# mehta-lab/VisCy

Hardware: AMD Instinct MI355X
Metric: training patches/sec (Z=5, 256x256, 1->2ch UNeXt2) (higher is better)
Workload: dtype bf16; 1 GPU; UNeXt2 2.5D convnextv2_tiny Z=5 256x256 1->2ch, fwd+MixedLoss(0.5,0,0.5)+bwd+AdamW; per_gpu_batch=512, global_batch=512, parallelism=dp1

## Files before the change

### include/vsx.h

```cpp
#ifndef VSX_H
#define VSX_H
#include <stddef.h>
#include <stdint.h>

#ifdef __cplusplus
extern "C" {
#endif

typedef void* vsx_stream_t;

#define VSX_F32 0
#define VSX_BF16 1

int32_t vsx_version(void);
const char* vsx_last_error(void);
const char* vsx_last_kernel(void);
int32_t vsx_set_flag(const char* name, int32_t value);
int32_t vsx_get_flag(const char* name);
int32_t vsx_det_workspace(float* ws, int64_t floats);
int32_t vsx_det_scope(int32_t on);
int32_t vsx_det_active(void);

#define VSX_A_ROWS 0
#define VSX_A_PATCH2 1
// ... 250 lines not shown
    float* dW2, float* db2, float* ws, int64_t ws_floats, int32_t nb, int32_t C, int32_t dtype, vsx_stream_t stream);
int64_t vsx_grn_q_reduce_ws_floats(int32_t nb, int32_t C);
int32_t vsx_mlp_bwd_stats(const void* dout, const void* wimg, const void* g, float* P, float* S, int64_t M, int32_t C, int32_t hw,
    int32_t dtype, vsx_stream_t stream);
int32_t vsx_mlp_bwd_dh(const void* dout, const void* wimg, const void* h, const float* s, const float* t, void* dh, float* ws,
                       int64_t ws_rows, float* colsum, const float* gelu_table, int64_t M, int32_t C, int32_t hw, int32_t dtype,
                       vsx_stream_t stream);
int32_t vsx_mlp_rows_per_workgroup(int32_t C, int32_t hw, int64_t M);
int32_t vsx_mlp_bwd_dh_re(const void* dout, const void* xh, const void* wimg_bwd, const void* wimg_fwd, const float* b1, const float* s,
                          const float* t, void* dh, float* ws, int64_t ws_rows, float* colsum, const float* gelu_table, int64_t M,
                          int32_t C, int32_t hw, int32_t dtype, vsx_stream_t stream);
int32_t vsx_mlp_bwd_dh_ln(const void* dout, const void* y, const float* mean, const float* rstd, const void* wimg_bwd,
                          const void* wimg_fwd, const float* b1, const float* s, const float* t, void* dh, float* ws, int64_t ws_rows,
                          float* colsum2, const float* gelu_table, int64_t M, int32_t C, int32_t hw, int32_t dtype,
                          vsx_stream_t stream);
int32_t vsx_mlp_gelu_table_len(void);
int32_t vsx_mlp_gelu_table(float* tab, vsx_stream_t stream);

int32_t vsx_adamw_advance(const double* cfg, int32_t* step, float* hyper, vsx_stream_t stream);

int32_t vsx_fill_f32(float* p, int64_t n, float value, vsx_stream_t stream);

int32_t vsx_prep_weight(const float* src, void* dst, void* dstT, const float* gamma, int32_t R, int32_t Cs,
    int32_t Tn, int32_t tapmode, int32_t dtype, vsx_stream_t stream);

int32_t vsx_unprep_grad(const float* g, float* dparam, const float* gamma, const float* W, float* dgamma,
    const float* u, const float* beta, const float* rowsub, int32_t R, int32_t Cs, int32_t Tn, int32_t tapmode,
    vsx_stream_t stream);

int32_t vsx_scale_weight_samples(const float* W, const float* s, void* out, int32_t B, int32_t R, int32_t K,
// ... 198 lines not shown
```

### viscy_amd/csrc/api.hip

```cpp
#include <stdarg.h>
#include <stdio.h>
#include <string.h>
#include "vsx_common.h"
#include "../../include/vsx.h"

static thread_local char g_err[512] = "";
thread_local const char* g_vsx_last_kernel = "";
int g_vsx_tn_tr = 1;
int g_vsx_nt_wide = 1;
int g_vsx_nt_fast = 3;
int g_vsx_tn_wide = 1;
int g_vsx_ggb_blocks = 2048;
int g_vsx_tn_rect = 11;
int g_vsx_dw_mfma = 15;
int g_vsx_ln_fblk = 32768;
int g_vsx_ln_bblk = 8192;
int g_vsx_ln_ablk = 512;
int g_vsx_ln_pack = 1;
int g_vsx_nt_stream = 3;
int g_vsx_grn_stream = 2;
int g_vsx_ggb_contig = 1;
int g_vsx_tn_fill = 1;
int g_vsx_tn_want2 = 512;
int g_vsx_tn_p2_rounds = 1;
// ... 56 lines not shown
    {"tn_want", &g_vsx_tn_want, INT32_MIN},       {"tn_p2_rounds", &g_vsx_tn_p2_rounds, INT32_MIN},
    {"tn_want2", &g_vsx_tn_want2, INT32_MIN},     {"tn_fill", &g_vsx_tn_fill, INT32_MIN},
    {"tn_contig", &g_vsx_tn_contig, INT32_MIN},   {"tn_stream", &g_vsx_tn_stream, INT32_MIN},
    {"ln_stream", &g_vsx_ln_stream, INT32_MIN},   {"ggb_blocks", &g_vsx_ggb_blocks, INT32_MIN},
    {"tn_rect", &g_vsx_tn_rect, INT32_MIN},       {"dw_mfma", &g_vsx_dw_mfma, INT32_MIN},
    {"ln_fblk", &g_vsx_ln_fblk, 1},               {"ln_bblk", &g_vsx_ln_bblk, 1},
    {"ln_ablk", &g_vsx_ln_ablk, 1},               {"ln_pack", &g_vsx_ln_pack, INT32_MIN},
    {"mlp_fused", &g_vsx_mlp_fused, INT32_MIN},   {"loss_fused", &g_vsx_loss_fused, INT32_MIN},
    {"mlp_sf32", &g_vsx_mlp_sf32, INT32_MIN},     {"det_reduce", &g_vsx_det_reduce, INT32_MIN},
    {"head_rows", &g_vsx_head_rows, INT32_MIN},   {"head_bps", &g_vsx_head_bps, 0},
};

extern "C" int32_t vsx_set_flag(const char* name, int32_t value) {
  for (const auto& f : g_flags)
    if (name && !strcmp(name, f.name) && value >= f.min) { *f.value = value; return 0; }
  vsx_set_error("vsx_set_flag: unknown flag '%s'", name ? name : "(null)");
  return 1;
}
extern "C" int32_t vsx_get_flag(const char* name) {
  for (const auto& f : g_flags)
    if (name && !strcmp(name, f.name)) return *f.value;
  return -1;
}
```

### viscy_amd/csrc/mlp.hip

```cpp
#include "vsx_common.h"
#include "mfma16.h"
#include "wtasks.h"
#include "../../include/vsx.h"

struct MlpArgs {
  const bf16_t* xh;
  const char* wimg;
  const float* b1;
  const float* grn_s;
  const float* grn_b;
  const float* b2;
  const bf16_t* res;
  const float* rscale;
  bf16_t* out;
  float* colsq;
  bf16_t* hout;
  bf16_t* gout;
  float ln_eps;
  bf16_t* xh_out;
  float* rstd_out;
  float* mean_out;
  const float* ln_mean;
  const float* ln_rstd;
  const bf16_t* tin;
  float* red0;
  float* red1;
  float* ws;
  const float* gtab;
  const bf16_t* xh2;
  const char* wimg2;
  int M, hw;
  int nt;
};

#define MLP_GT_BASE (103 << 7)
#define MLP_GT_LIM (131 << 7)
#define MLP_GT_N (MLP_GT_LIM - MLP_GT_BASE)

__device__ __forceinline__ float mlp_relu(float h) {
  const int b = __float_as_int(h);
  return __int_as_float(b > 0 ? b : 0);
}

__device__ __forceinline__ uint32_t mlp_relu_pair(uint32_t w) {
  typedef short mlp_s16x2 __attribute__((ext_vector_type(2)));
  const mlp_s16x2 z = {0, 0};
  return __builtin_bit_cast(uint32_t, __builtin_elementwise_max(__builtin_bit_cast(mlp_s16x2, w), z));
// ... 3 lines not shown
__device__ unsigned long long g_mlp_ts[8 * 64 * 8];
#define MLP_STAMP(k) do { if (blockIdx.x == gridDim.x / 2 + 7 && lane == 0) g_mlp_ts[(wave * 64 + hs) * 8 + (k)] = __builtin_amdgcn_s_memtime(); } while (0)
#else
#define MLP_STAMP(k) do { } while (0)
#endif

#ifndef MLP_DMA_WAVES
#define MLP_DMA_WAVES 4
#endif

template <int C, int MF, int NW, int MODE>
struct MlpGeom {
  static constexpr int H4 = 4 * C, NHS = H4 / 32, KK = C / 32, NF = C / 16;
  static constexpr int WM = 16 * MF, BM = NW * WM;
  static constexpr int W1_PIECES = 2 * KK, IMG_PIECES = 2 * KK + NF;
  static constexpr bool RE = MODE == 5 || MODE == 7;
  static constexpr int NP = RE ? 2 * W1_PIECES : (MODE != 1 ? W1_PIECES : IMG_PIECES);
  static constexpr int STAGE_BYTES = NP * 1024;
  static constexpr int OB_COLS = MODE == 0 ? 32 : 64;
  static constexpr int OB_RS = OB_COLS * 2 + 16;
  static constexpr int OUT_BYTES = MODE == 2 ? NW * 2 * WM * OB_RS : NW * WM * OB_RS;
  static constexpr bool B1_IN_PADS = MODE == 6;
  static constexpr int VEC_FLOATS = MODE == 1 ? 3 * H4 + C : (MODE == 4 ? 2 * H4 : (RE ? 3 * H4 : (MODE == 3 || B1_IN_PADS ? 4 : H4)));
  static constexpr int RED_FLOATS = MODE == 1 ? 4 : (MODE == 3 || MODE == 7 ? 4 * NW * 32 : 2 * NW * 32);
  static constexpr int GT_FLOATS = (MODE <= 2 || MODE == 6) ? MLP_GT_N : ((MODE == 4 || RE) ? 2 * MLP_GT_N : 4);
  static constexpr int LDS_BYTES = 2 * STAGE_BYTES + OUT_BYTES + (VEC_FLOATS + RED_FLOATS) * 4;
};

template <int C, int MF, int NW, int MODE>
__device__ __forceinline__ void mlp_fused_body(const MlpArgs& a) {
  typedef MlpGeom<C, MF, NW, MODE> G;
  constexpr int H4 = G::H4, NHS = G::NHS, KK = G::KK, NF = G::NF, WM = G::WM;
  constexpr bool STATS = MODE == 0 || MODE == 2 || MODE == 6, STORE = MODE == 2 || MODE == 6, STORE_H = MODE == 2;
  constexpr bool RE = G::RE, LNF = MODE == 7;
  constexpr bool BWD = (MODE >= 3 && MODE <= 5) || MODE == 7, DH = MODE == 4 || RE;
  constexpr int DW = MLP_DMA_WAVES < NW ? MLP_DMA_WAVES : NW;
  __shared__ __attribute__((aligned(1024))) char buf0[G::STAGE_BYTES];
  __shared__ __attribute__((aligned(1024))) char buf1[G::STAGE_BYTES];
  __shared__ __attribute__((aligned(16))) float vec[G::VEC_FLOATS];
  __shared__ __attribute__((aligned(16))) float red[G::RED_FLOATS];
  __shared__ __attribute__((aligned(16))) char obuf[G::OUT_BYTES];
  __shared__ __attribute__((aligned(16))) float gt[G::GT_FLOATS];

  const int tid = threadIdx.x;
  const MfLane ln = mf_lane(tid);
  const int lane = ln.lane, wave = ln.wave, p16 = ln.p16, kq = ln.kq;
  const int m0 = blockIdx.x * G::BM;
  const int b = m0 / a.hw;
  const int row0 = m0 + wave * WM;

// ... 66 lines not shown
  mf_bf16x8 xf[MF][KK];
#pragma unroll
  for (int mf = 0; mf < MF; ++mf)
#pragma unroll
    for (int kk = 0; kk < KK; ++kk)
      xf[mf][kk] = *reinterpret_cast<const mf_bf16x8*>(a.xh + (size_t)(row0 + mf * 16 + p16) * C + kk * 32 + kq * 8);

  mf_bf16x8 xg[RE ? MF : 1][RE ? KK : 1];
  if constexpr (RE) {
#pragma unroll
    for (int mf = 0; mf < MF; ++mf)
#pragma unroll
      for (int kk = 0; kk < KK; ++kk)
        xg[mf][kk] = *reinterpret_cast<const mf_bf16x8*>(a.xh2 + (size_t)(row0 + mf * 16 + p16) * C + kk * 32 + kq * 8);
  }
  setup_to_lds();
  float rsr[LNF ? MF : 1];
  mf_bf16x8 wS, wSl, wMh, wMl;
  if constexpr (LNF) {
#pragma unroll
    for (int mf = 0; mf < MF; ++mf) {
      const size_t rowi = (size_t)(row0 + mf * 16 + p16);
      const float mean = a.ln_mean[rowi], rstd = a.ln_rstd[rowi];
      rsr[mf] = rstd;
#pragma unroll
      for (int kk = 0; kk < KK; ++kk) {
        union { mf_bf16x8 b; uint4 u; } cv;
        cv.b = xg[mf][kk];
        float v[8], o[8];
        unpack<bf16_t>(cv.u, v);
// ... 63 lines not shown
          }
        }
        if constexpr (STORE) {
          if (kq == 0) {
            a.rstd_out[rowi] = rstd;
            if (a.mean_out) a.mean_out[rowi] = mean;
          }
        }
      }
    }
  }

  mf_f32x4 oacc[MODE == 1 ? MF : 1][MODE == 1 ? NF : 1];
  if constexpr (MODE == 1) {
    mfma_zero(oacc);
  }

  auto gemm1 = [&](const char* W, const auto& xfr, mf_f32x4 (&acc)[2][MF]) {
    mfma_zero(acc);
#pragma unroll
    for (int hf = 0; hf < 2; ++hf)
#pragma unroll
      for (int kk = 0; kk < KK; ++kk) {
        const mf_bf16x8 wa = *reinterpret_cast<const mf_bf16x8*>(W + (hf * KK + kk) * 1024);
#pragma unroll
        for (int mf = 0; mf < MF; ++mf) acc[hf][mf] = mfma16(wa, xfr[mf][kk], acc[hf][mf]);
      }
  };
  char* sb = obuf + wave * ((STORE_H ? 2 : 1) * WM * G::OB_RS);
  auto activate = [&](int hs, const mf_f32x4 (&acc)[2][MF], mf_bf16x8 (&zf)[MF]) {
// ... 120 lines not shown
  };
  auto tile_flush = [&](int hs) {
    if constexpr (DH) {
      __builtin_amdgcn_fence(__ATOMIC_RELEASE, "wavefront");
      __builtin_amdgcn_wave_barrier();
#pragma unroll
      for (int i = 0; i < (WM * 8) / 64; ++i) {
        const int idx = lane + 64 * i, row = idx >> 3, ch = idx & 7;
        const uint4 v = *reinterpret_cast<const uint4*>(sb + row * G::OB_RS + ch * 16);
        stvec_stream(a.hout + (size_t)(row0 + row) * H4 + (hs - 1) * 32 + ch * 8, v, (a.nt & 1) != 0);
      }
      __builtin_amdgcn_fence(__ATOMIC_RELEASE, "wavefront");
      __builtin_amdgcn_wave_barrier();
    }
  };
  auto bwd_act = [&](int hs, const mf_f32x4 (&acc)[2][MF], const mf_f32x4 (&hacc)[2][MF], float (&r0)[2][4], float (&r1)[2][4]) {
    if constexpr (BWD) {
#pragma unroll
      for (int hf = 0; hf < 2; ++hf)
#pragma unroll
        for (int r = 0; r < 4; ++r) { r0[hf][r] = 0.f; r1[hf][r] = 0.f; }
      float sv[2][4], tv[2][4], b1v[2][4];
      if constexpr (DH) {
        const float* vb = vec + hs * 32 + kq * 4;
#pragma unroll
        for (int hf = 0; hf < 2; ++hf) {
          const float4 t2 = *reinterpret_cast<const float4*>(vb + hf * 16);
          const float4 t3 = *reinterpret_cast<const float4*>(vb + H4 + hf * 16);
          sv[hf][0] = t2.x; sv[hf][1] = t2.y; sv[hf][2] = t2.z; sv[hf][3] = t2.w;
          tv[hf][0] = t3.x; tv[hf][1] = t3.y; tv[hf][2] = t3.z; tv[hf][3] = t3.w;
          if constexpr (RE) {
            const float4 t4 = *reinterpret_cast<const float4*>(vb + 2 * H4 + hf * 16);
            b1v[hf][0] = t4.x; b1v[hf][1] = t4.y; b1v[hf][2] = t4.z; b1v[hf][3] = t4.w;
          }
        }
      }
#pragma unroll
      for (int mf = 0; mf < MF; ++mf)
#pragma unroll
        for (int hf = 0; hf < 2; ++hf) {
          char* tp = sb + (mf * 16 + p16) * G::OB_RS + ((hs & 1) * 32 + hf * 16 + kq * 4) * 2;
          uint2 tw;
          if constexpr (RE) {
            const vsx_v2f ha = (vsx_v2f){hacc[hf][mf][0], hacc[hf][mf][1]} + (vsx_v2f){b1v[hf][0], b1v[hf][1]};
            const vsx_v2f hc = (vsx_v2f){hacc[hf][mf][2], hacc[hf][mf][3]} + (vsx_v2f){b1v[hf][2], b1v[hf][3]};
            tw.x = f32x2_to_bf16x2_bits(ha.x, ha.y);
            tw.y = f32x2_to_bf16x2_bits(hc.x, hc.y);
          } else {
            tw = *reinterpret_cast<const uint2*>(tp);
          }
          if constexpr (MODE == 3) {
            const float e[4] = {__uint_as_float(tw.x << 16), __uint_as_float(tw.x & 0xFFFF0000u), __uint_as_float(tw.y << 16),
                                __uint_as_float(tw.y & 0xFFFF0000u)};
// ... 16 lines not shown
#pragma unroll
            for (int r = 0; r < 4; r += 2) {
              const uint32_t w = r < 2 ? tw.x : tw.y;
              const float h0 = __uint_as_float(w << 16), h1 = __uint_as_float(w & 0xFFFF0000u);
              const vsx_v2f d2 = {acc[hf][mf][r], acc[hf][mf][r + 1]};
              const vsx_v2f s2 = {sv[hf][r], sv[hf][r + 1]}, t2 = {tv[hf][r], tv[hf][r + 1]};
              const uint32_t Rq = mlp_relu_pair(w);
              const vsx_v2f gv = (vsx_v2f){__uint_as_float(Rq << 16), __uint_as_float(Rq & 0xFFFF0000u)} - (vsx_v2f){tb[r].x, tb[r + 1].x};
              const vsx_v2f cs = {copysignf(tb[r].y, h0), copysignf(tb[r + 1].y, h1)};
              const vsx_v2f dgv = cs + (vsx_v2f){0.5f, 0.5f};
              vsx_v2f rr = (d2 * s2 + gv * t2) * dgv;
              if constexpr (LNF) rr = rr * (vsx_v2f){rsr[mf], rsr[mf]};
              ob[r / 2] = f32x2_to_bf16x2_bits(rr.x, rr.y);
            }
            *reinterpret_cast<uint2*>(tp) = make_uint2(ob[0], ob[1]);
          }
        }
    }
  };

  auto stage_load2 = [&](int s, char* dst) {
    const char* src1 = a.wimg + (size_t)(s + 1) * (G::IMG_PIECES * 1024) + lane * 16;
    const char* src2 = RE ? a.wimg2 + (size_t)(s + 1) * (G::IMG_PIECES * 1024) - G::W1_PIECES * 1024 + lane * 16
                          : a.wimg + (size_t)s * (G::IMG_PIECES * 1024) + lane * 16;
    if (wave >= DW) return;
    for (int p = wave; p < G::NP; p += DW) {
      if ((RE || p < G::W1_PIECES) && s + 1 >= NHS) continue;
      const char* src = p < G::W1_PIECES ? src1 : src2;
      lds_dma16(src + p * 1024, dst + p * 1024);
    }
  };
  auto store_pending = [&](int hs) {
    if constexpr (STORE) {
      __builtin_amdgcn_fence(__ATOMIC_RELEASE, "wavefront");
      __builtin_amdgcn_wave_barrier();
      for (int idx = lane; idx < (STORE_H ? 2 : 1) * WM * 8; idx += 64) {
        const int o = idx / (WM * 8), rem = idx - o * (WM * 8);
        const int row = rem >> 3, ch = rem & 7;
        const uint4 v = *reinterpret_cast<const uint4*>(sb + (o * WM + row) * G::OB_RS + ch * 16);
        bf16_t* dst = (o || !STORE_H ? a.gout : a.hout) + (size_t)(row0 + row) * H4 + (hs - 1) * 32 + ch * 8;
        stvec_stream(dst, v, (a.nt & 1) != 0);
// ... 75 lines not shown
    }
    mf_bf16x8 zf[MF];
    __builtin_amdgcn_sched_barrier(0);
    MLP_STAMP(2);
    gemm1(S, xf, hnxt);
    if constexpr (RE) gemm1(S + G::W1_PIECES * 1024, xg, gnxt);
    __builtin_amdgcn_sched_group_barrier(0x100, 3, 0);
#pragma unroll
    for (int i = 0; i < (RE ? 4 : 2) * KK; ++i) {
      __builtin_amdgcn_sched_group_barrier(0x008, MF, 0);
      __builtin_amdgcn_sched_group_barrier(0x100, 1, 0);
    }
    __builtin_amdgcn_sched_barrier(0);
    MLP_STAMP(3);
    float q0[2][4], q1[2][4];
    if constexpr (RE) bwd_act(hs, hcur, gcur, q0, q1);
    else if constexpr (BWD) bwd_act(hs, hcur, hcur, q0, q1);
    else activate(hs, hcur, zf);
    __builtin_amdgcn_sched_barrier(0);
    MLP_STAMP(4);
    if constexpr (DH) {
      colsum_mfma(hs, red + (hs & 1) * (LNF ? 2 : 1) * NW * 32 + wave * 32);
    } else if constexpr (BWD) {
      float* rw = red + (hs & 1) * 2 * NW * 32 + wave * 32;
#pragma unroll
      for (int hf = 0; hf < 2; ++hf)
#pragma unroll
        for (int r = 0; r < 4; ++r) {
          const float t0 = group_sum<16>(q0[hf][r]);
          if (p16 == 0) rw[hf * 16 + kq * 4 + r] = t0;
          const float t1 = group_sum<16>(q1[hf][r]);
          if (p16 == 0) rw[NW * 32 + hf * 16 + kq * 4 + r] = t1;
        }
    } else if constexpr (STATS) {
      stats_mfma(hs, red + (hs & 1) * NW * 32 + wave * 32);
// ... 43 lines not shown

  if constexpr (BWD) {
    tile_flush(NHS - 1);
    __syncthreads();
    if constexpr (MODE == 3) {
      if (wave == (NHS - 1) % DW) {
        const float* r = red + ((NHS - 1) & 1) * 2 * NW * 32 + (lane >> 5) * NW * 32 + (lane & 31);
        float t = 0.f;
#pragma unroll
        for (int w = 0; w < NW; ++w) t += r[w * 32];
        atomicAdd((lane < 32 ? a.red0 : a.red1) + (size_t)b * H4 + (NHS - 1) * 32 + (lane & 31), t);
      }
    } else {
      ws_row(NHS - 1, true);
    }
    return;
  } else if constexpr (STATS) {
    store_pending(NHS - 1);
    __syncthreads();
    if (wave == (NHS - 1) % DW && lane < 32) {
      const float* r = red + ((NHS - 1) & 1) * NW * 32 + lane;
      float t = 0.f;
#pragma unroll
      for (int w = 0; w < NW; ++w) t += r[w * 32];
      if (a.ws) a.ws[(size_t)blockIdx.x * H4 + (NHS - 1) * 32 + lane] = t;
      else atomicAdd(a.colsq + (size_t)b * H4 + (NHS - 1) * 32 + lane, t);
    }
    return;
  } else {
    const float rs = a.rscale ? a.rscale[b] : 1.f;
// ... 55 lines not shown
__global__ __launch_bounds__(NW * 64, (MODE == 4 && NW == 8 && C == 96 ? 4 : 1)) void mlp_fused_kernel(const MlpArgs a) {
  mlp_fused_body<C, MF, NW, MODE>(a);
}
template <int C, int MF, int NW, int MODE>
__global__ __launch_bounds__(NW * 64, (MODE == 4 && NW == 8 && C == 96 ? 4 : 1)) __attribute__((target("no-packed-fp32-ops")))
void mlp_fused_kernel_sf(const MlpArgs a) {
  mlp_fused_body<C, MF, NW, MODE>(a);
}

__global__ __launch_bounds__(256) void mlp_pack_kernel(const bf16_t* __restrict__ W1, const bf16_t* __restrict__ W2,
                                                       char* __restrict__ img, int C) {
  wt_mlp_pack(blockIdx.x, W1, W2, img, C);
}

struct MlpCfg { int C, MF, NW, modes; };
static inline int mlp_nt() { return (g_vsx_nt_stream >> 2) & 15; }
static const MlpCfg kMlpCfgs[] = {{96, 2, 8, 255}, {192, 2, 8, 255}, {224, 2, 8, 255}, {384, 2, 8, 4 | 8 | 16}};

static const MlpCfg* mlp_cfg(int C, int hw, long M, int mode) {
  for (const MlpCfg& c : kMlpCfgs) {
    const int bm = c.NW * 16 * c.MF;
    if (!(c.modes & (1 << mode))) continue;
    if (c.C == 384 && !(g_vsx_mlp_fused & 4)) continue;
    if ((mode == 5 || mode == 6 || mode == 7) && !(g_vsx_mlp_fused & 64)) continue;
    if (mode == 7 && !(g_vsx_mlp_fused & 128)) continue;
    if (c.C == C && hw % bm == 0 && M % bm == 0) return &c;
  }
  return nullptr;
}

extern "C" int32_t vsx_mlp_supported(int32_t C, int32_t hw, int64_t M, int32_t dtype) {
  return dtype == VSX_BF16 && mlp_cfg(C, hw, M, 0) != nullptr && mlp_cfg(C, hw, M, 1) != nullptr;
}
extern "C" int32_t vsx_mlp_mode_supported(int32_t C, int32_t hw, int64_t M, int32_t mode, int32_t dtype) {
  return dtype == VSX_BF16 && mode >= 0 && mode <= 7 && mlp_cfg(C, hw, M, mode) != nullptr;
}

extern "C" int64_t vsx_mlp_image_bytes(int32_t C) { return (int64_t)(4 * C / 32) * (2 * (C / 32) + C / 16) * 1024; }

extern "C" int32_t vsx_mlp_pack(const void* W1, const void* W2, void* img, int32_t C, vsx_stream_t stream) {
  VSX_CHECK(W1 && W2 && img && C > 0 && C % 32 == 0, "vsx_mlp_pack: bad arguments (C = %d must be a multiple of 32)", C);
  const long total = (long)(4 * C / 32) * (2 * (C / 32) + C / 16) * 64;
  hipLaunchKernelGGL(mlp_pack_kernel, dim3(vsx_cdiv(total, 256)), dim3(256), 0, (hipStream_t)stream, (const bf16_t*)W1,
                     (const bf16_t*)W2, (char*)img, C);
  VSX_LAUNCH_CHECK();
  return 0;
}

template <int C, int MF, int NW, int MODE>
static int mlp_launch(const MlpArgs& a, hipStream_t s) {
  typedef MlpGeom<C, MF, NW, MODE> G;
  if (g_vsx_mlp_sf32 & (1 << MODE)) hipLaunchKernelGGL((mlp_fused_kernel_sf<C, MF, NW, MODE>), dim3(a.M / G::BM), dim3(NW * 64), 0, s, a);
  else hipLaunchKernelGGL((mlp_fused_kernel<C, MF, NW, MODE>), dim3(a.M / G::BM), dim3(NW * 64), 0, s, a);
  VSX_LAUNCH_CHECK();
  return 0;
}

template <int MODE>
static int mlp_dispatch(const MlpCfg* c, const MlpArgs& a, hipStream_t s) {
  if (c->C == 96) return mlp_launch<96, 2, 8, MODE>(a, s);
  if (c->C == 192) return mlp_launch<192, 2, 8, MODE>(a, s);
  if (c->C == 224) return mlp_launch<224, 2, 8, MODE>(a, s);
  if constexpr (MODE <= 1 || MODE >= 5) { vsx_set_error("vsx_mlp: mode %d is built for C <= 224", MODE); return 1; }
  else return mlp_launch<384, 2, 8, MODE>(a, s);
}

static long mlp_det_need(const MlpCfg* c, long M) { return M / (c->NW * 16 * c->MF) * 4 * c->C; }
static int mlp_det_begin(MlpArgs& a, const MlpCfg* c, const char* who) { return vsx_det_take(who, mlp_det_need(c, a.M), &a.ws); }
static int mlp_det_end(const MlpArgs& a, const MlpCfg* c, hipStream_t s) {
  if (!a.ws) return 0;
  const int bm = c->NW * 16 * c->MF;
  return vsx_det_group_sum(a.ws, 4 * c->C, 0, a.colsq, a.M / a.hw, a.hw / bm, 4 * c->C, s);
}

extern "C" int32_t vsx_mlp_gelu_table_len(void) { return 2 * MLP_GT_N; }

__global__ void mlp_gelu_table_kernel(float* __restrict__ tab) {
// ... 132 lines not shown
  return mlp_bwd_dh_run<5>("vsx_mlp_bwd_dh_re", a, s, t, dh, ws, ws_rows, colsum, 4 * C, gtab, M, C, hw, stream);
}

extern "C" int32_t vsx_mlp_bwd_dh_ln(const void* dout, const void* y, const float* mean, const float* rstd, const void* wimg_bwd,
                                     const void* wimg_fwd, const float* b1, const float* s, const float* t, void* dh, float* ws,
                                     int64_t ws_rows, float* colsum2, const float* gtab, int64_t M, int32_t C, int32_t hw,
                                     int32_t dtype, vsx_stream_t stream) {
  VSX_CHECK(dtype == VSX_BF16, "vsx_mlp_bwd_dh_ln: bf16 only");
  VSX_CHECK(dout && y && mean && rstd && wimg_bwd && wimg_fwd && b1 && s && t && dh && ws && colsum2 && gtab && M > 0 && hw > 0,
            "vsx_mlp_bwd_dh_ln: bad arguments");
  MlpArgs a = mlp_bwd_args(dout, wimg_bwd, M, hw);
  a.xh2 = (const bf16_t*)y; a.wimg2 = (const char*)wimg_fwd; a.b1 = b1; a.ln_mean = mean; a.ln_rstd = rstd;
  return mlp_bwd_dh_run<7>("vsx_mlp_bwd_dh_ln", a, s, t, dh, ws, ws_rows, colsum2, 8 * C, gtab, M, C, hw, stream);
}

#ifdef MLP_TS
extern "C" int32_t vsx_debug_mlp_ts(unsigned long long* host_out) {
  return hipMemcpyFromSymbol(host_out, HIP_SYMBOL(g_mlp_ts), sizeof(g_mlp_ts)) == hipSuccess ? 0 : 1;
}
#endif

extern "C" int64_t vsx_mlp_det_floats(int32_t C, int32_t hw, int64_t M, int32_t mode) {
  const MlpCfg* c = mode == 0 || mode == 2 || mode == 6 ? mlp_cfg(C, hw, M, mode) : nullptr;
  return c ? mlp_det_need(c, M) : 0;
}

extern "C" int32_t vsx_mlp_rows_per_workgroup(int32_t C, int32_t hw, int64_t M) {
  const MlpCfg* c = mlp_cfg(C, hw, M, 4);
  return c ? c->NW * 16 * c->MF : 0;
}
// ... 1 lines not shown
```

### viscy_amd/csrc/vsx_common.h

```cpp
#pragma once
#include <hip/hip_runtime.h>
#include <stdint.h>
#include <math.h>
#include <type_traits>

typedef __bf16 bf16_t;

#define VSX_F32 0
#define VSX_BF16 1

void vsx_set_error(const char* fmt, ...);
extern int g_vsx_tn_tr, g_vsx_tn_wide, g_vsx_tn_rect, g_vsx_tn_want, g_vsx_tn_want2, g_vsx_tn_p2_rounds, g_vsx_tn_fill, g_vsx_tn_contig, g_vsx_tn_stream;
extern int g_vsx_nt_wide, g_vsx_nt_fast, g_vsx_nt_stream, g_vsx_nt2;
extern int g_vsx_ln_fblk, g_vsx_ln_bblk, g_vsx_ln_ablk, g_vsx_ln_pack, g_vsx_ln_stream;
extern int g_vsx_grn_stream, g_vsx_ggb_contig, g_vsx_ggb_blocks;
extern int g_vsx_dw_mfma, g_vsx_mlp_fused, g_vsx_mlp_sf32, g_vsx_loss_fused;
extern int g_vsx_head_bps, g_vsx_head_rows, g_vsx_det_reduce;
extern thread_local int g_vsx_det_scope;
static inline bool vsx_det_on() { return g_vsx_det_reduce || g_vsx_det_scope; }
int vsx_det_take(const char* who, long need, float** ws);
int vsx_det_group_sum(const float* ws, int ld, int col0, float* out, int groups, int rows_per_group, int N, hipStream_t s);
extern thread_local const char* g_vsx_last_kernel;
#define VSX_CHECK(cond, ...)            \
  do {                                  \
    if (!(cond)) {                      \
      vsx_set_error(__VA_ARGS__);       \
      return 1;                         \
    }                                   \
  } while (0)
#define VSX_LAUNCH_CHECK()                                               \
  do {                                                                   \
    hipError_t e_ = hipGetLastError();                                   \
// ... 239 lines not shown
```

### viscy_amd/engine_unext2.py

```python

from __future__ import annotations

import os
from collections import namedtuple
from typing import NamedTuple

import torch
from torch import Tensor

from . import _lib as L
from . import ops as hip_ops
from .flat import FlatEngine, engine_apply


class _BlockW:

    __slots__ = ("C", "p", "dw_w", "W1f", "W1fT", "b1f", "W2", "W2T", "v1", "fc2_w", "fc2_b", "grn_w", "grn_b", "dp", "img", "img2", "b2f")


class _ProjW:
    __slots__ = ("cin", "cout", "taps", "ln", "conv", "W", "WT")


FWD_UNFUSED, FWD_PAIR, FWD_FC1 = 0, 1, 2
# ... 67 lines not shown
            self.off += n_al
            return v
        return self._zeros(*shape)


class Engine(FlatEngine):
    name = "UNeXt2"

    def __init__(self, model, ops=None):
        ops = hip_ops if ops is None else ops
        self._hip = ops is hip_ops
        self._mlp_flag = 0
        self.cfg = model.cfg
        self._zeros4c = {}
        self._dp_inject = None
        self._za = None
        self._za_need = {}
        self._prepared_for = None
        self.W = None
        super().__init__(model, ops)

    def _stage_params_rev(self, stage):
        ps = []
        for blk in reversed(list(stage.blocks)):
            if hasattr(blk, "gamma"):
                ps += [blk.gamma, blk.mlp.fc2.weight, blk.mlp.fc2.bias, blk.mlp.fc1.weight, blk.mlp.fc1.bias, blk.norm.weight,
                       blk.norm.bias, blk.conv_dw.weight, blk.conv_dw.bias]
                continue
            ps += [blk.mlp.fc2.weight, blk.mlp.fc2.bias, blk.mlp.grn.weight, blk.mlp.grn.bias, blk.mlp.fc1.weight,
                   blk.mlp.fc1.bias, blk.norm.weight, blk.norm.bias, blk.conv_dw.weight, blk.conv_dw.bias]
# ... 75 lines not shown
        w = _ProjW()
        cout, cin = conv.weight.shape[0], conv.weight.shape[1]
        taps = conv.weight.shape[2] * conv.weight.shape[3]
        w.cin, w.cout, w.taps, w.ln, w.conv = cin, cout, taps, ln, conv
        if cout < 16:
            w.W = w.WT = None
        else:
            w.W, w.WT = o.prep_weight(conv.weight, cout, cin, taps, dt, want=True, want_t=need_bwd)
        return w

    def prepare(self, dt: torch.dtype, need_bwd: bool, mlp_flag: int = 0):
        key = (dt, need_bwd)
        m, cfg, o = self.model, self.cfg, self.ops
        with o.batch():
            W = self._prepare_ops(dt, need_bwd)
        if dt == torch.bfloat16 and mlp_flag:
            bwd_img = need_bwd and bool(mlp_flag & 8)
            with o.batch():
                for _, blocks in list(W["enc"]) + list(W["dec"]):
                    for w in blocks:
                        if any(o.mlp_supported(w.C, 1 << 20, 1 << 20, dt, md) for md in (None, 2, 4)):
                            w.img = o.mlp_pack(w.W1f, w.W2, w.C)
                            if bwd_img:
                                w.img2 = o.mlp_pack(w.W2T, w.W2, w.C)
        self.W = W
        self._prepared_for = key
        return W

    def _prepare_ops(self, dt: torch.dtype, need_bwd: bool):
        m, cfg, o = self.model, self.cfg, self.ops
        W = {"dt": dt}
        sw = m.stem.conv.weight
        co3, K = sw.shape[0], sw[0].numel()
        Dp = cfg["ratio"]
        narrow_stem = cfg.get("head") == "shuffle" and tuple(cfg["stem_kernel"][1:]) == (2, 2)
        if narrow_stem and K % 8 and Dp == 1:
            W["stem_W"], W["stem_b"] = None, m.stem.conv.bias
        elif Dp == 1:
            W["stem_W"], _ = o.prep_weight(sw, co3, K, 1, dt)
# ... 213 lines not shown
                o.transpose_f32(cs, db2, C, 1, True)
            o.matvec_t_add(w.fc2_w, cs, dgb, C, 4 * C)
        else:
            o.gemm("tn", gact, dout, dW2, M, C, 4 * C, 4 * C, C, 4 * C, dtype=dt, pro=L.PRO_GRN, grn_s=s,
                   grn_b=w.grn_b, hw=hw, colsum=db2)
        if w.v1:
            o.layer_scale_unfold(dW2, db2, blk.mlp.fc2.weight, blk.mlp.fc2.bias, blk.gamma, g(blk.mlp.fc2.weight),
                                 g(blk.mlp.fc2.bias), g(blk.gamma))
        ln_re = not plan.keep_xh
        u1 = None
        if ln_re:
            cs2 = self._za.take(2, 4 * C)
            db1f, u1 = cs2[0], cs2[1]
        else:
            db1f = self._za.take(4 * C)
        if fused_bwd:
            img2 = w.img2
            assert img2 is not None
            if fused_bwd == 2 and not stats_in_tn:
                o.mlp_bwd_stats(dout, img2, gact, PS[0], PS[1], M, C, hw)
            if stats_in_tn:
                t = o.grn_bwd_stats(colsq, PS[0], w.grn_w, dgw)
            else:
                t = o.grn_bwd_stats(colsq, PS[0], w.grn_w, dgw, Sb=PS[1], dbeta=dgb)
            if ln_re:
                dz = o.mlp_bwd_dh_ln(dout, y, mean, rstd, img2, w.img, w.b1f, s, t, cs2, M, C, hw)
            elif not plan.keep_h:
                dz = o.mlp_bwd_dh_re(dout, xh, img2, w.img, w.b1f, s, t, db1f, M, C, hw)
            else:
                dz = o.mlp_bwd_dh(dout, img2, h, s, t, db1f, M, C, hw)
        else:
            dz = torch.empty((M, 4 * C), dtype=dt, device=dev)
            o.gemm("nt", dout, w.W2T, dz, M, 4 * C, C, C, C, 4 * C, dtype=dt, epi=L.EPI_DZ, aux=gact, ldx=4 * C, red0=PS[0],
                   red1=PS[1], hw=hw)
            t = o.grn_bwd_stats(colsq, PS[0], w.grn_w, dgw, Sb=PS[1], dbeta=dgb)
            o.grn_gelu_bwd(dz, h, s, t, db1f, M, 4 * C, hw)
        if ln_re:
            xh = y
        dy = o.dgrad_ln_bwd(dz, w.W1fT, xh, rstd, M, C, 4 * C, mean=mean) if self._hip else None
        assert dy is not None or not ln_re
        dxh = None
        if dy is None:
            dxh = torch.empty((M, C), dtype=dt, device=dev)
            o.gemm("nt", dz, w.W1fT, dxh, M, C, 4 * C, 4 * C, 4 * C, C, dtype=dt)
        dW1f = self._za.take(4 * C, C)
        o.gemm("tn", xh, dz, dW1f, M, 4 * C, C, C, 4 * C, C, dtype=dt)
        del dz
        o.unprep_grad(dW1f, g(blk.mlp.fc1.weight), 4 * C, C, 1, gamma=blk.norm.weight, W=blk.mlp.fc1.weight,
                      dgamma=g(blk.norm.weight), u=db1f, beta=blk.norm.bias, rowsub=u1)
        o.matvec_t_add(blk.mlp.fc1.weight, db1f, g(blk.norm.bias), 4 * C, C)
        o.transpose_f32(db1f, g(blk.mlp.fc1.bias), 4 * C, 1, True)
        if dy is None:
            dy = o.ln_bwd(dxh, xh, None, rstd, None, None, None, None, M, C)
        del dxh
# ... 380 lines not shown
```

### viscy_amd/ops.py

```python

from __future__ import annotations

import contextlib
import ctypes as C
import os
import threading
from typing import Sequence

import torch
from torch import Tensor

from . import _lib as L
from ._lib import VsxGemm, VsxGemmPlan, check, dtype_code, lib, ptr, stream


class Scratch:

    def __init__(self, alloc=None):
        self._alloc = alloc or (lambda floats, dev: torch.empty(floats, dtype=torch.float32, device=dev))
        self._tls = threading.local()
        self.held: list = []

    def take(self, dev, floats: int):
        arenas = getattr(self._tls, "arenas", None)
# ... 524 lines not shown
def mlp_bwd_dh(dout: Tensor, img2: Tensor, h: Tensor, s: Tensor, t: Tensor, colsum: Tensor, M: int, C: int, hw: int) -> Tensor:
    dh, ws, rows = _mlp_dh_alloc(dout, M, C, hw, 4 * C)
    check(lib().vsx_mlp_bwd_dh(ptr(dout), ptr(img2), ptr(h), ptr(s), ptr(t), ptr(dh), ptr(ws), rows, ptr(colsum),
                               ptr(_gelu_table(dout.device)), M, C, hw, dtype_code(dout.dtype), stream()), "mlp_bwd_dh")
    return dh


def mlp_bwd_dh_re(dout: Tensor, xh: Tensor, img2: Tensor, img: Tensor, b1: Tensor, s: Tensor, t: Tensor, colsum: Tensor, M: int, C: int,
                  hw: int) -> Tensor:
    dh, ws, rows = _mlp_dh_alloc(dout, M, C, hw, 4 * C)
    check(lib().vsx_mlp_bwd_dh_re(ptr(dout), ptr(xh), ptr(img2), ptr(img), ptr(b1), ptr(s), ptr(t), ptr(dh), ptr(ws), rows, ptr(colsum),
                                  ptr(_gelu_table(dout.device)), M, C, hw, dtype_code(dout.dtype), stream()), "mlp_bwd_dh_re")
    return dh


def mlp_bwd_dh_ln(dout: Tensor, y: Tensor, mean: Tensor, rstd: Tensor, img2: Tensor, img: Tensor, b1: Tensor, s: Tensor, t: Tensor,
                  colsum2: Tensor, M: int, C: int, hw: int) -> Tensor:
    dh, ws, rows = _mlp_dh_alloc(dout, M, C, hw, 8 * C)
    check(lib().vsx_mlp_bwd_dh_ln(ptr(dout), ptr(y), ptr(mean), ptr(rstd), ptr(img2), ptr(img), ptr(b1), ptr(s), ptr(t), ptr(dh), ptr(ws),
                                  rows, ptr(colsum2), ptr(_gelu_table(dout.device)), M, C, hw, dtype_code(dout.dtype), stream()),
          "mlp_bwd_dh_ln")
    return dh


def mlp_out(xh: Tensor, img: Tensor, b1: Tensor, s: Tensor, beta: Tensor, b2: Tensor, res: Tensor, rscale: Tensor | None,
            M: int, C: int, hw: int, ln_eps: float = 0.0) -> Tensor:
    out = torch.empty((M, C), dtype=xh.dtype, device=xh.device)
    _mlp_fwd("mlp_out", 1, xh, ln_eps, img, b1, s, beta, b2, res, rscale, out, None, M=M, C=C, hw=hw)
    return out

# ... 841 lines not shown
```

Baseline: 5601 patches/s.

## Fuse fc1 dgrad and LayerNorm backward into the MLP dh kernel for C=96

Adds a new fused MLP backward mode (8) that, while it computes dh, also accumulates dh·W1ᵀ with MFMA using a third weight image staged in LDS. At the end of the kernel it applies the LayerNorm backward (rstd, row means of d and d·x) and writes dy directly. This removes the separate dgrad_ln_bwd GEMM and its re-read of dz for the C=96 blocks. The cost is extra LDS staging, extra accumulator registers (NF×MF) and more per-wave epilogue work, which could lower occupancy. It is enabled by default through a new dh_dgrad switch, and img2 is repacked with W1fT in place of W2 when it is on.

```diff
diff --git a/include/vsx.h b/include/vsx.h
--- a/include/vsx.h
+++ b/include/vsx.h
@@ -288,6 +288,10 @@
                           const void* wimg_fwd, const float* b1, const float* s, const float* t, void* dh, float* ws, int64_t ws_rows,
                           float* colsum2, const float* gelu_table, int64_t M, int32_t C, int32_t hw, int32_t dtype,
                           vsx_stream_t stream);
+int32_t vsx_mlp_bwd_dh_dgrad(const void* dout, const void* xh, const float* rstd, const void* wimg_bwd, const void* wimg_fwd,
+                             const void* wimg_dg, const float* b1, const float* s, const float* t, void* dh, void* dy, float* ws,
+                             int64_t ws_rows, float* colsum, const float* gelu_table, int64_t M, int32_t C, int32_t hw, int32_t dtype,
+                             vsx_stream_t stream);
 int32_t vsx_mlp_gelu_table_len(void);
 int32_t vsx_mlp_gelu_table(float* tab, vsx_stream_t stream);
 
diff --git a/viscy_amd/csrc/api.hip b/viscy_amd/csrc/api.hip
--- a/viscy_amd/csrc/api.hip
+++ b/viscy_amd/csrc/api.hip
@@ -94,11 +94,14 @@
 extern "C" int32_t vsx_set_flag(const char* name, int32_t value) {
   for (const auto& f : g_flags)
     if (name && !strcmp(name, f.name) && value >= f.min) { *f.value = value; return 0; }
+  if (int* sw = name ? vsx_mlp_switch(name) : nullptr)
+    if (value == 0 || value == 1) { *sw = value; return 0; }
   vsx_set_error("vsx_set_flag: unknown flag '%s'", name ? name : "(null)");
   return 1;
 }
 extern "C" int32_t vsx_get_flag(const char* name) {
   for (const auto& f : g_flags)
     if (name && !strcmp(name, f.name)) return *f.value;
+  if (const int* sw = name ? vsx_mlp_switch(name) : nullptr) return *sw;
   return -1;
 }
diff --git a/viscy_amd/csrc/mlp.hip b/viscy_amd/csrc/mlp.hip
--- a/viscy_amd/csrc/mlp.hip
+++ b/viscy_amd/csrc/mlp.hip
@@ -1,3 +1,4 @@
+#include <string.h>
 #include "vsx_common.h"
 #include "mfma16.h"
 #include "wtasks.h"
@@ -31,6 +32,7 @@
   const char* wimg2;
   int M, hw;
   int nt;
+  const char* wimg3;
 };
 
 #define MLP_GT_BASE (103 << 7)
@@ -64,8 +66,9 @@
   static constexpr int H4 = 4 * C, NHS = H4 / 32, KK = C / 32, NF = C / 16;
   static constexpr int WM = 16 * MF, BM = NW * WM;
   static constexpr int W1_PIECES = 2 * KK, IMG_PIECES = 2 * KK + NF;
-  static constexpr bool RE = MODE == 5 || MODE == 7;
-  static constexpr int NP = RE ? 2 * W1_PIECES : (MODE != 1 ? W1_PIECES : IMG_PIECES);
+  static constexpr bool RE = MODE == 5 || MODE == 7 || MODE == 8;
+  static constexpr bool DG = MODE == 8;
+  static constexpr int NP = RE ? 2 * W1_PIECES + (DG ? NF : 0) : (MODE != 1 ? W1_PIECES : IMG_PIECES);
   static constexpr int STAGE_BYTES = NP * 1024;
   static constexpr int OB_COLS = MODE == 0 ? 32 : 64;
   static constexpr int OB_RS = OB_COLS * 2 + 16;
@@ -82,8 +85,8 @@
   typedef MlpGeom<C, MF, NW, MODE> G;
   constexpr int H4 = G::H4, NHS = G::NHS, KK = G::KK, NF = G::NF, WM = G::WM;
   constexpr bool STATS = MODE == 0 || MODE == 2 || MODE == 6, STORE = MODE == 2 || MODE == 6, STORE_H = MODE == 2;
-  constexpr bool RE = G::RE, LNF = MODE == 7;
-  constexpr bool BWD = (MODE >= 3 && MODE <= 5) || MODE == 7, DH = MODE == 4 || RE;
+  constexpr bool RE = G::RE, LNF = MODE == 7, DG = G::DG;
+  constexpr bool BWD = (MODE >= 3 && MODE <= 5) || MODE == 7 || DG, DH = MODE == 4 || RE;
   constexpr int DW = MLP_DMA_WAVES < NW ? MLP_DMA_WAVES : NW;
   __shared__ __attribute__((aligned(1024))) char buf0[G::STAGE_BYTES];
   __shared__ __attribute__((aligned(1024))) char buf1[G::STAGE_BYTES];
@@ -180,6 +183,11 @@
       for (int kk = 0; kk < KK; ++kk)
         xg[mf][kk] = *reinterpret_cast<const mf_bf16x8*>(a.xh2 + (size_t)(row0 + mf * 16 + p16) * C + kk * 32 + kq * 8);
   }
+  float rsd[DG ? MF : 1];
+  if constexpr (DG) {
+#pragma unroll
+    for (int mf = 0; mf < MF; ++mf) rsd[mf] = a.ln_rstd[(size_t)(row0 + mf * 16 + p16)];
+  }
   setup_to_lds();
   float rsr[LNF ? MF : 1];
   mf_bf16x8 wS, wSl, wMh, wMl;
@@ -273,6 +281,10 @@
   mf_f32x4 oacc[MODE == 1 ? MF : 1][MODE == 1 ? NF : 1];
   if constexpr (MODE == 1) {
     mfma_zero(oacc);
+  }
+  mf_f32x4 dacc[DG ? NF : 1][DG ? MF : 1];
+  if constexpr (DG) {
+    mfma_zero(dacc);
   }
 
   auto gemm1 = [&](const char* W, const auto& xfr, mf_f32x4 (&acc)[2][MF]) {
@@ -423,7 +435,8 @@
       __builtin_amdgcn_wave_barrier();
     }
   };
-  auto bwd_act = [&](int hs, const mf_f32x4 (&acc)[2][MF], const mf_f32x4 (&hacc)[2][MF], float (&r0)[2][4], float (&r1)[2][4]) {
+  auto bwd_act = [&](int hs, const mf_f32x4 (&acc)[2][MF], const mf_f32x4 (&hacc)[2][MF], float (&r0)[2][4], float (&r1)[2][4],
+                     mf_bf16x8 (&dhf)[DG ? MF : 1]) {
     if constexpr (BWD) {
 #pragma unroll
       for (int hf = 0; hf < 2; ++hf)
@@ -445,7 +458,8 @@
         }
       }
 #pragma unroll
-      for (int mf = 0; mf < MF; ++mf)
+      for (int mf = 0; mf < MF; ++mf) {
+        uint32_t dq[4];
 #pragma unroll
         for (int hf = 0; hf < 2; ++hf) {
           char* tp = sb + (mf * 16 + p16) * G::OB_RS + ((hs & 1) * 32 + hf * 16 + kq * 4) * 2;
@@ -492,8 +506,11 @@
               ob[r / 2] = f32x2_to_bf16x2_bits(rr.x, rr.y);
             }
             *reinterpret_cast<uint2*>(tp) = make_uint2(ob[0], ob[1]);
-          }
-        }
+            if constexpr (DG) { dq[hf * 2] = ob[0]; dq[hf * 2 + 1] = ob[1]; }
+          }
+        }
+        if constexpr (DG) dhf[mf] = __builtin_bit_cast(mf_bf16x8, make_uint4(dq[0], dq[1], dq[2], dq[3]));
+      }
     }
   };
 
@@ -503,6 +520,12 @@
                           : a.wimg + (size_t)s * (G::IMG_PIECES * 1024) + lane * 16;
     if (wave >= DW) return;
     for (int p = wave; p < G::NP; p += DW) {
+      if constexpr (DG) {
+        if (p >= 2 * G::W1_PIECES) {
+          lds_dma16(a.wimg3 + ((size_t)s * G::IMG_PIECES + p - G::W1_PIECES) * 1024 + lane * 16, dst + p * 1024);
+          continue;
+        }
+      }
       if ((RE || p < G::W1_PIECES) && s + 1 >= NHS) continue;
       const char* src = p < G::W1_PIECES ? src1 : src2;
       lds_dma16(src + p * 1024, dst + p * 1024);
@@ -608,11 +631,20 @@
     __builtin_amdgcn_sched_barrier(0);
     MLP_STAMP(3);
     float q0[2][4], q1[2][4];
-    if constexpr (RE) bwd_act(hs, hcur, gcur, q0, q1);
-    else if constexpr (BWD) bwd_act(hs, hcur, hcur, q0, q1);
+    mf_bf16x8 dhf[DG ? MF : 1];
+    if constexpr (RE) bwd_act(hs, hcur, gcur, q0, q1, dhf);
+    else if constexpr (BWD) bwd_act(hs, hcur, hcur, q0, q1, dhf);
     else activate(hs, hcur, zf);
     __builtin_amdgcn_sched_barrier(0);
     MLP_STAMP(4);
+    if constexpr (DG) {
+#pragma unroll
+      for (int nf = 0; nf < NF; ++nf) {
+        const mf_bf16x8 wa = *reinterpret_cast<const mf_bf16x8*>(S + (2 * G::W1_PIECES + nf) * 1024);
+#pragma unroll
+        for (int mf = 0; mf < MF; ++mf) dacc[nf][mf] = mfma16(wa, dhf[mf], dacc[nf][mf]);
+      }
+    }
     if constexpr (DH) {
       colsum_mfma(hs, red + (hs & 1) * (LNF ? 2 : 1) * NW * 32 + wave * 32);
     } else if constexpr (BWD) {
@@ -686,6 +718,71 @@
     } else {
       ws_row(NHS - 1, true);
     }
+    if constexpr (DG) {
+      const float invC = 1.f / (float)C;
+      uint2 dyq[MF][NF];
+#pragma unroll
+      for (int mf = 0; mf < MF; ++mf) {
+        char* trow = sb + (mf * 16 + p16) * G::OB_RS;
+        float xa[NF][4];
+#pragma unroll
+        for (int cb = 0; cb < KK; cb += 2) {
+#pragma unroll
+          for (int kk = cb; kk < cb + 2 && kk < KK; ++kk)
+            *reinterpret_cast<uint4*>(trow + ((kk - cb) * 32 + kq * 8) * 2) = __builtin_bit_cast(uint4, xg[mf][kk]);
+          __builtin_amdgcn_fence(__ATOMIC_RELEASE, "wavefront");
+          __builtin_amdgcn_wave_barrier();
+#pragma unroll
+          for (int nf = cb * 2; nf < cb * 2 + 4 && nf < NF; ++nf) {
+            const uint2 t = *reinterpret_cast<const uint2*>(trow + ((nf - cb * 2) * 16 + kq * 4) * 2);
+            xa[nf][0] = __uint_as_float(t.x << 16); xa[nf][1] = __uint_as_float(t.x & 0xFFFF0000u);
+            xa[nf][2] = __uint_as_float(t.y << 16); xa[nf][3] = __uint_as_float(t.y & 0xFFFF0000u);
+          }
+          __builtin_amdgcn_fence(__ATOMIC_RELEASE, "wavefront");
+          __builtin_amdgcn_wave_barrier();
+        }
+        float d[NF][4], s1 = 0.f, s2 = 0.f;
+#pragma unroll
+        for (int nf = 0; nf < NF; ++nf)
+#pragma unroll
+          for (int r = 0; r < 4; ++r) {
+            d[nf][r] = round_bf16(dacc[nf][mf][r]);
+            s1 += d[nf][r];
+            s2 = fmaf(d[nf][r], xa[nf][r], s2);
+          }
+        s1 += __shfl_xor(s1, 16, 64); s1 += __shfl_xor(s1, 32, 64);
+        s2 += __shfl_xor(s2, 16, 64); s2 += __shfl_xor(s2, 32, 64);
+        const float rs = rsd[mf];
+        const float m1 = s1 * invC, m2 = s2 * invC;
+#pragma unroll
+        for (int nf = 0; nf < NF; ++nf) {
+          float o[4];
+#pragma unroll
+          for (int r = 0; r < 4; ++r) o[r] = rs * (d[nf][r] - m1 - xa[nf][r] * m2);
+          dyq[mf][nf] = make_uint2(f32x2_to_bf16x2_bits(o[0], o[1]), f32x2_to_bf16x2_bits(o[2], o[3]));
+        }
+      }
+      bf16_t* orow = a.out + (size_t)row0 * C;
+#pragma unroll
+      for (int cb = 0; cb < NF; cb += 4) {
+        const int nfe = cb + 4 < NF ? cb + 4 : NF;
+#pragma unroll
+        for (int mf = 0; mf < MF; ++mf)
+#pragma unroll
+          for (int nf = cb; nf < cb + 4 && nf < NF; ++nf)
+            *reinterpret_cast<uint2*>(sb + (mf * 16 + p16) * G::OB_RS + ((nf - cb) * 16 + kq * 4) * 2) = dyq[mf][nf];
+        __builtin_amdgcn_fence(__ATOMIC_RELEASE, "wavefront");
+        __builtin_amdgcn_wave_barrier();
+        const int chs = (nfe - cb) * 2;
+        for (int idx = lane; idx < WM * chs; idx += 64) {
+          const int row = idx / chs, ch = idx - row * chs;
+          const uint4 v = *reinterpret_cast<const uint4*>(sb + row * G::OB_RS + ch * 16);
+          *reinterpret_cast<uint4*>(orow + (size_t)row * C + cb * 16 + ch * 8) = v;
+        }
+        __builtin_amdgcn_fence(__ATOMIC_RELEASE, "wavefront");
+        __builtin_amdgcn_wave_barrier();
+      }
+    }
     return;
   } else if constexpr (STATS) {
     store_pending(NHS - 1);
@@ -771,15 +868,18 @@
 }
 
 struct MlpCfg { int C, MF, NW, modes; };
+static int s_dh_dgrad = 1;
+int* vsx_mlp_switch(const char* name) { return !strcmp(name, "dh_dgrad") ? &s_dh_dgrad : nullptr; }
+
 static inline int mlp_nt() { return (g_vsx_nt_stream >> 2) & 15; }
-static const MlpCfg kMlpCfgs[] = {{96, 2, 8, 255}, {192, 2, 8, 255}, {224, 2, 8, 255}, {384, 2, 8, 4 | 8 | 16}};
+static const MlpCfg kMlpCfgs[] = {{96, 2, 8, 255 | 256}, {192, 2, 8, 255}, {224, 2, 8, 255}, {384, 2, 8, 4 | 8 | 16}};
 
 static const MlpCfg* mlp_cfg(int C, int hw, long M, int mode) {
   for (const MlpCfg& c : kMlpCfgs) {
     const int bm = c.NW * 16 * c.MF;
     if (!(c.modes & (1 << mode))) continue;
     if (c.C == 384 && !(g_vsx_mlp_fused & 4)) continue;
-    if ((mode == 5 || mode == 6 || mode == 7) && !(g_vsx_mlp_fused & 64)) continue;
+    if ((mode == 5 || mode == 6 || mode == 7 || mode == 8) && !(g_vsx_mlp_fused & 64)) continue;
     if (mode == 7 && !(g_vsx_mlp_fused & 128)) continue;
     if (c.C == C && hw % bm == 0 && M % bm == 0) return &c;
   }
@@ -790,7 +890,7 @@
   return dtype == VSX_BF16 && mlp_cfg(C, hw, M, 0) != nullptr && mlp_cfg(C, hw, M, 1) != nullptr;
 }
 extern "C" int32_t vsx_mlp_mode_supported(int32_t C, int32_t hw, int64_t M, int32_t mode, int32_t dtype) {
-  return dtype == VSX_BF16 && mode >= 0 && mode <= 7 && mlp_cfg(C, hw, M, mode) != nullptr;
+  return dtype == VSX_BF16 && mode >= 0 && mode <= 8 && mlp_cfg(C, hw, M, mode) != nullptr;
 }
 
 extern "C" int64_t vsx_mlp_image_bytes(int32_t C) { return (int64_t)(4 * C / 32) * (2 * (C / 32) + C / 16) * 1024; }
@@ -816,8 +916,9 @@
 template <int MODE>
 static int mlp_dispatch(const MlpCfg* c, const MlpArgs& a, hipStream_t s) {
   if (c->C == 96) return mlp_launch<96, 2, 8, MODE>(a, s);
-  if (c->C == 192) return mlp_launch<192, 2, 8, MODE>(a, s);
-  if (c->C == 224) return mlp_launch<224, 2, 8, MODE>(a, s);
+  if constexpr (MODE == 8) { vsx_set_error("vsx_mlp: mode 8 is built for C = 96"); return 1; }
+  else if (c->C == 192) return mlp_launch<192, 2, 8, MODE>(a, s);
+  else if (c->C == 224) return mlp_launch<224, 2, 8, MODE>(a, s);
   if constexpr (MODE <= 1 || MODE >= 5) { vsx_set_error("vsx_mlp: mode %d is built for C <= 224", MODE); return 1; }
   else return mlp_launch<384, 2, 8, MODE>(a, s);
 }
@@ -980,6 +1081,18 @@
   return mlp_bwd_dh_run<7>("vsx_mlp_bwd_dh_ln", a, s, t, dh, ws, ws_rows, colsum2, 8 * C, gtab, M, C, hw, stream);
 }
 
+extern "C" int32_t vsx_mlp_bwd_dh_dgrad(const void* dout, const void* xh, const float* rstd, const void* wimg_bwd, const void* wimg_fwd,
+                                        const void* wimg_dg, const float* b1, const float* s, const float* t, void* dh, void* dy,
+                                        float* ws, int64_t ws_rows, float* colsum, const float* gtab, int64_t M, int32_t C, int32_t hw,
+                                        int32_t dtype, vsx_stream_t stream) {
+  VSX_CHECK(dtype == VSX_BF16, "vsx_mlp_bwd_dh_dgrad: bf16 only");
+  VSX_CHECK(dout && xh && rstd && wimg_bwd && wimg_fwd && wimg_dg && b1 && s && t && dh && dy && ws && colsum && gtab && M > 0 && hw > 0,
+            "vsx_mlp_bwd_dh_dgrad: bad arguments");
+  MlpArgs a = mlp_bwd_args(dout, wimg_bwd, M, hw);
+  a.xh2 = (const bf16_t*)xh; a.wimg2 = (const char*)wimg_fwd; a.wimg3 = (const char*)wimg_dg; a.b1 = b1; a.ln_rstd = rstd; a.out = (bf16_t*)dy;
+  return mlp_bwd_dh_run<8>("vsx_mlp_bwd_dh_dgrad", a, s, t, dh, ws, ws_rows, colsum, 4 * C, gtab, M, C, hw, stream);
+}
+
 #ifdef MLP_TS
 extern "C" int32_t vsx_debug_mlp_ts(unsigned long long* host_out) {
   return hipMemcpyFromSymbol(host_out, HIP_SYMBOL(g_mlp_ts), sizeof(g_mlp_ts)) == hipSuccess ? 0 : 1;
diff --git a/viscy_amd/csrc/vsx_common.h b/viscy_amd/csrc/vsx_common.h
--- a/viscy_amd/csrc/vsx_common.h
+++ b/viscy_amd/csrc/vsx_common.h
@@ -16,6 +16,7 @@
 extern int g_vsx_grn_stream, g_vsx_ggb_contig, g_vsx_ggb_blocks;
 extern int g_vsx_dw_mfma, g_vsx_mlp_fused, g_vsx_mlp_sf32, g_vsx_loss_fused;
 extern int g_vsx_head_bps, g_vsx_head_rows, g_vsx_det_reduce;
+int* vsx_mlp_switch(const char* name);
 extern thread_local int g_vsx_det_scope;
 static inline bool vsx_det_on() { return g_vsx_det_reduce || g_vsx_det_scope; }
 int vsx_det_take(const char* who, long need, float** ws);
diff --git a/viscy_amd/engine_unext2.py b/viscy_amd/engine_unext2.py
--- a/viscy_amd/engine_unext2.py
+++ b/viscy_amd/engine_unext2.py
@@ -105,6 +105,7 @@
         self.cfg = model.cfg
         self._zeros4c = {}
         self._dp_inject = None
+        self._dh_dgrad = False
         self._za = None
         self._za_need = {}
         self._prepared_for = None
@@ -210,15 +211,18 @@
         m, cfg, o = self.model, self.cfg, self.ops
         with o.batch():
             W = self._prepare_ops(dt, need_bwd)
+        self._dh_dgrad = False
         if dt == torch.bfloat16 and mlp_flag:
             bwd_img = need_bwd and bool(mlp_flag & 8)
+            self._dh_dgrad = bwd_img and bool(L.lib().vsx_get_flag(b"dh_dgrad"))
             with o.batch():
                 for _, blocks in list(W["enc"]) + list(W["dec"]):
                     for w in blocks:
                         if any(o.mlp_supported(w.C, 1 << 20, 1 << 20, dt, md) for md in (None, 2, 4)):
                             w.img = o.mlp_pack(w.W1f, w.W2, w.C)
                             if bwd_img:
-                                w.img2 = o.mlp_pack(w.W2T, w.W2, w.C)
+                                dg = self._dh_dgrad and o.mlp_supported(w.C, 1 << 20, 1 << 20, dt, 8)
+                                w.img2 = o.mlp_pack(w.W2T, w.W1fT if dg else w.W2, w.C)
         self.W = W
         self._prepared_for = key
         return W
@@ -462,6 +466,7 @@
             db1f, u1 = cs2[0], cs2[1]
         else:
             db1f = self._za.take(4 * C)
+        dy = None
         if fused_bwd:
             img2 = w.img2
             assert img2 is not None
@@ -473,6 +478,8 @@
                 t = o.grn_bwd_stats(colsq, PS[0], w.grn_w, dgw, Sb=PS[1], dbeta=dgb)
             if ln_re:
                 dz = o.mlp_bwd_dh_ln(dout, y, mean, rstd, img2, w.img, w.b1f, s, t, cs2, M, C, hw)
+            elif not plan.keep_h and self._dh_dgrad and o.mlp_supported(C, hw, M, dt, 8):
+                dz, dy = o.mlp_bwd_dh_dgrad(dout, xh, rstd, img2, w.img, img2, w.b1f, s, t, db1f, M, C, hw)
             elif not plan.keep_h:
                 dz = o.mlp_bwd_dh_re(dout, xh, img2, w.img, w.b1f, s, t, db1f, M, C, hw)
             else:
@@ -485,7 +492,8 @@
             o.grn_gelu_bwd(dz, h, s, t, db1f, M, 4 * C, hw)
         if ln_re:
             xh = y
-        dy = o.dgrad_ln_bwd(dz, w.W1fT, xh, rstd, M, C, 4 * C, mean=mean) if self._hip else None
+        if dy is None:
+            dy = o.dgrad_ln_bwd(dz, w.W1fT, xh, rstd, M, C, 4 * C, mean=mean) if self._hip else None
         assert dy is not None or not ln_re
         dxh = None
         if dy is None:
diff --git a/viscy_amd/ops.py b/viscy_amd/ops.py
--- a/viscy_amd/ops.py
+++ b/viscy_amd/ops.py
@@ -562,6 +562,16 @@
     return dh
 
 
+def mlp_bwd_dh_dgrad(dout: Tensor, xh: Tensor, rstd: Tensor, img2: Tensor, img: Tensor, img_dg: Tensor, b1: Tensor, s: Tensor, t: Tensor,
+                     colsum: Tensor, M: int, C: int, hw: int) -> tuple[Tensor, Tensor]:
+    dh, ws, rows = _mlp_dh_alloc(dout, M, C, hw, 4 * C)
+    dy = torch.empty((M, C), dtype=dout.dtype, device=dout.device)
+    check(lib().vsx_mlp_bwd_dh_dgrad(ptr(dout), ptr(xh), ptr(rstd), ptr(img2), ptr(img), ptr(img_dg), ptr(b1), ptr(s), ptr(t), ptr(dh),
+                                     ptr(dy), ptr(ws), rows, ptr(colsum), ptr(_gelu_table(dout.device)), M, C, hw,
+                                     dtype_code(dout.dtype), stream()), "mlp_bwd_dh_dgrad")
+    return dh, dy
+
+
 def mlp_bwd_dh_ln(dout: Tensor, y: Tensor, mean: Tensor, rstd: Tensor, img2: Tensor, img: Tensor, b1: Tensor, s: Tensor, t: Tensor,
                   colsum2: Tensor, M: int, C: int, hw: int) -> Tensor:
     dh, ws, rows = _mlp_dh_alloc(dout, M, C, hw, 8 * C)
```

New measurement: 5651 patches/s, median of 6. No clear change (+0.9%).
